# Allenxuxu/gev

Measured on AMD Instinct MI355X. Metric: GiB/s WS payload unmasked (device-resident) + frames/s, 64 KiB masked frames, higher is better.
Workload: dtype u8

## Files before the change

### gev_amd/csrc/gevws_kernels.hpp

```cpp
#pragma once

#include <hip/hip_runtime.h>

#include <cstdint>
#include <cstdio>
#include <cstring>

#include "gevws.h"

typedef uint32_t u32x4 __attribute__((ext_vector_type(4)));
typedef uint64_t u64x2 __attribute__((ext_vector_type(2)));

namespace {

constexpr int kWalkBlock = 256;
constexpr int kCountBlock = 64;
constexpr int kScanBlock = 1024;
constexpr int kUnmaskBlock = 256;
constexpr uint64_t kTile = GEVWS_TILE;
static_assert(kTile == kUnmaskBlock * 16, "one tile = one 16-byte chunk per lane");
constexpr int kBlkFields = 4;
constexpr int kDecFields = 5;
constexpr uint32_t kFusedScanMaxBlocks = 256;
constexpr size_t kWalkPartBytes = (size_t)kFusedScanMaxBlocks * kDecFields * 2 * sizeof(uint64_t);
// ... 269 lines not shown
constexpr uint32_t kSmallConns = 256;
constexpr uint64_t kSmallBytes = 64 * 1024;
constexpr uint32_t kOneLaunchConns = GEVWS_ONE_LAUNCH_MAX_CONNS;
constexpr uint64_t kOneLaunchBytes = GEVWS_ONE_LAUNCH_MAX_BYTES;
static_assert(kOneLaunchConns == 1024 && kOneLaunchBytes == 128 * 1024, "k_decode_small's wide shape");
__device__ __forceinline__ uint64_t gpu_ticks() { return __builtin_amdgcn_s_memrealtime(); }
__device__ __forceinline__ void signal_done(uint32_t* done, uint32_t seq, uint64_t* ticks = nullptr, uint64_t t0 = 0,
                                            int slot = 0) {
  if (!done) return;
  if (ticks && threadIdx.x == 0) {
    ticks[2 * slot] = t0;
    ticks[2 * slot + 1] = gpu_ticks();
  }
  __threadfence_system();
  __syncthreads();
  if (threadIdx.x == 0) __hip_atomic_store(done, seq, __ATOMIC_RELEASE, __HIP_MEMORY_SCOPE_SYSTEM);
}

constexpr uint64_t kSplitMinBytes = 16384;
constexpr uint32_t kSplitMaxLanes = 32;
constexpr uint64_t kSplitLanesPerCU = 512;

constexpr uint64_t kBigFrameBytes = 48 * 1024;
constexpr uint32_t kWideGridPerCU = 32;
constexpr uint64_t kWideGridTiles = 2ull << 20;
constexpr uint32_t kUnmaskRunCounters = 8;
constexpr uint64_t kUnmaskRun = 16;
constexpr uint64_t kUnmaskRunMinTiles = 64;

__device__ __forceinline__ uint32_t active_groups(uint64_t total, uint64_t nframes, uint32_t big_grid,
                                                  bool wide = false) {
  const uint32_t ncu = big_grid & 0xffffu, norm = big_grid >> 16;
  if (ncu == 0 || gridDim.x <= ncu || nframes == 0) return gridDim.x;
  if (total / nframes >= kBigFrameBytes) return ncu;
  return (norm == 0 || wide || gridDim.x <= norm) ? gridDim.x : norm;
}

template <bool NT>
__device__ __forceinline__ u32x4 ld16u_stream(const uint8_t* p) {
  if constexpr (NT) {
    return __builtin_nontemporal_load(reinterpret_cast<const u32x4*>(p));
  } else {
    return ld16u(p);
  }
}

__device__ __forceinline__ void st16_nt(uint8_t* p, u32x4 x) {
  __builtin_nontemporal_store(x, reinterpret_cast<u32x4*>(p));
}

constexpr int kWinTiles = 4;

__device__ __forceinline__ u32x4 rot_next_lane(u32x4 x) {
  return u32x4{(uint32_t)__builtin_amdgcn_update_dpp(0, (int)x[0], 0x134, 0xf, 0xf, false),
               (uint32_t)__builtin_amdgcn_update_dpp(0, (int)x[1], 0x134, 0xf, 0xf, false),
               (uint32_t)__builtin_amdgcn_update_dpp(0, (int)x[2], 0x134, 0xf, 0xf, false),
               (uint32_t)__builtin_amdgcn_update_dpp(0, (int)x[3], 0x134, 0xf, 0xf, false)};
}

__device__ __forceinline__ u32x4 funnel16(u32x4 a, u32x4 b, uint32_t m) {
  const uint32_t r = m & 3;
  u32x4 o;
  switch (m >> 2) {
    case 0:
      o = u32x4{__builtin_amdgcn_alignbyte(a[1], a[0], r), __builtin_amdgcn_alignbyte(a[2], a[1], r),
                __builtin_amdgcn_alignbyte(a[3], a[2], r), __builtin_amdgcn_alignbyte(b[0], a[3], r)};
      break;
    case 1:
      o = u32x4{__builtin_amdgcn_alignbyte(a[2], a[1], r), __builtin_amdgcn_alignbyte(a[3], a[2], r),
                __builtin_amdgcn_alignbyte(b[0], a[3], r), __builtin_amdgcn_alignbyte(b[1], b[0], r)};
      break;
    case 2:
      o = u32x4{__builtin_amdgcn_alignbyte(a[3], a[2], r), __builtin_amdgcn_alignbyte(b[0], a[3], r),
                __builtin_amdgcn_alignbyte(b[1], b[0], r), __builtin_amdgcn_alignbyte(b[2], b[1], r)};
      break;
    default:
      o = u32x4{__builtin_amdgcn_alignbyte(b[0], a[3], r), __builtin_amdgcn_alignbyte(b[1], b[0], r),
                __builtin_amdgcn_alignbyte(b[2], b[1], r), __builtin_amdgcn_alignbyte(b[3], b[2], r)};
      break;
  }
  return o;
}

}
```

### gev_amd/csrc/gevws_unmask.hip

```cpp
#include "gevws_internal.hpp"

namespace {

__device__ __forceinline__ uint64_t find_frame(const gevws_frame* __restrict__ frames,
                                               const uint32_t* __restrict__ tile_first, uint64_t t,
                                               uint64_t ntiles, uint64_t nframes, uint64_t p) {
  uint64_t lo = tile_first[t];
  uint64_t hi = (t + 1 < ntiles) ? (uint64_t)tile_first[t + 1] : nframes - 1;
  while (lo < hi) {
    const uint64_t mid = (lo + hi + 1) >> 1;
    if (frames[mid].payload_off <= p) lo = mid; else hi = mid - 1;
  }
  return lo;
}

__device__ __forceinline__ void unmask_chunk_lookup(const uint8_t* __restrict__ in,
                                                    const gevws_frame* __restrict__ frames,
                                                    const uint32_t* __restrict__ tile_first, uint64_t t,
                                                    uint64_t ntiles, uint64_t nframes, uint64_t p,
                                                    uint8_t* __restrict__ out) {
  const gevws_frame* fr = frames + find_frame(frames, tile_first, t, ntiles, nframes, p);
  const uint64_t rel = p - fr->payload_off;
  uint32_t k;
  memcpy(&k, fr->hdr.mask, 4);
// ... 155 lines not shown
    const uint64_t wbase = base;
    const uint64_t f_lo = tile_first[t];
    const uint64_t f_hi = wend_t < ntiles ? (uint64_t)tile_first[wend_t] : nframes - 1;
    const uint64_t F = f_hi - f_lo + 1;
    if (F <= (uint64_t)kWinFrames) {
      __syncthreads();
      for (uint64_t i = threadIdx.x; i < F; i += kUnmaskBlock) {
        const uint64_t* rec = reinterpret_cast<const uint64_t*>(frames + f_lo + i);
        const uint64_t w0 = rec[0];
        const uint64_t Ln = rec[1];
        const uint64_t po = rec[2];
        const uint64_t so = rec[3];
        s_start[i] = po > wbase ? (uint32_t)(po - wbase) : 0u;
        const uint64_t lend = po + Ln;
        s_lend[i] = lend <= wbase ? 0 : (lend - wbase > 0x7fffffffull ? 0x7fffffff : (int32_t)(lend - wbase));
        s_delta[i] = so - po;
        s_key[i] = ((w0 >> 24) & 0xff) ? (uint32_t)(w0 >> 32) : 0u;
      }
      __syncthreads();
      u32x4 v[WT];
      uint32_t key[WT];
      int32_t rem[WT];
#pragma unroll
      for (int u = 0; u < WT; ++u) {
        const uint32_t rel = (uint32_t)(u * kTile) + lane_off;
        const uint64_t p = wbase + rel;
        rem[u] = 0;
        key[u] = 0;
        v[u] = u32x4{0, 0, 0, 0};
        if ((uint64_t)u < wt && p < total) {
          uint32_t lo = 0, hi = (uint32_t)F - 1;
          while (lo < hi) {
            const uint32_t mid = (lo + hi + 1) >> 1;
            if (s_start[mid] <= rel) lo = mid; else hi = mid - 1;
          }
          rem[u] = s_lend[lo] - (int32_t)rel;
          key[u] = s_key[lo];
          v[u] = ld16u_stream<true>(in + (p + s_delta[lo]));
        }
      }
#pragma unroll
      for (int u = 0; u < WT; ++u) {
        if (rem[u] > 0) {
          u32x4 x = v[u] ^ key[u];
          if (rem[u] < 16) x = keep_bytes(x, rem[u]);
          st16_nt(out + wbase + (uint32_t)(u * kTile) + lane_off, x);
        }
      }
      t = wend_t;
      continue;
    }
    const uint64_t p = base + lane_off;
    if (p < total) unmask_chunk_lookup(in, frames, tile_first, t, ntiles, nframes, p, out);
    t += 1;
  }
  if (!dyn) break;
  }
}

constexpr int kWin5Frames = 1024;
constexpr uint32_t kWinChunks = 8 * (uint32_t)kTile / 16;
constexpr uint32_t kQuarter = kWinChunks / (kUnmaskBlock / 64);
constexpr uint32_t kTmapN = 512;

struct WinRec {
  u64x2 lo;
  u64x2 hi;
};

__device__ __forceinline__ WinRec load_rec(const gevws_frame* __restrict__ frames, uint64_t f) {
  const u64x2* r = reinterpret_cast<const u64x2*>(frames + f);
  return WinRec{r[0], r[1]};
}

struct WinLds5 {
  int32_t* lend;
  uint64_t* delta;
  uint32_t* key;
  uint16_t* own;
  uint32_t* wtot;
  uint32_t* tmap;
};

template <int U>
__device__ __forceinline__ void unmask_v5_body(const uint8_t* __restrict__ in, const gevws_frame* __restrict__ frames,
                                               const uint32_t* __restrict__ tile_first,
                                               const gevws_summary* __restrict__ sum, uint8_t* __restrict__ out,
                                               uint32_t big_grid, const WinLds5& L, bool wide = false,
                                               uint32_t* __restrict__ runs = nullptr) {
  constexpr int WT = 8;
  static_assert(WT * kTile / 16 == kWinChunks && kWinChunks == 8 * kUnmaskBlock, "8 chunks per thread");
  if (sum->status != GEVWS_OK) return;
  const uint64_t total = sum->payload_bytes;
  const uint64_t nframes = sum->frames;
  const uint64_t ntiles = (total + kTile - 1) / kTile;
  const uint32_t groups = active_groups(total, nframes, big_grid, wide);
  if (blockIdx.x >= groups) return;
  const uint64_t per = (ntiles + groups - 1) / groups;
  const bool dyn = runs != nullptr && groups >= kUnmaskRunCounters;
  uint64_t t = dyn ? 0 : (uint64_t)blockIdx.x * per;
  uint64_t tend = dyn ? 0 : (t + per < ntiles ? t + per : ntiles);
  const uint32_t xc = blockIdx.x % kUnmaskRunCounters;
  const uint64_t segn = ((ntiles + kUnmaskRunCounters - 1) / kUnmaskRunCounters + kUnmaskRun - 1) / kUnmaskRun * kUnmaskRun;
  const uint64_t seg0 = xc * segn < ntiles ? xc * segn : ntiles;
  const uint64_t seg1 = seg0 + segn < ntiles ? seg0 + segn : ntiles;
  {
    const uint32_t tid = fresh_tid();
    reinterpret_cast<u32x4*>(L.own)[tid] = u32x4{0, 0, 0, 0};
    reinterpret_cast<u32x4*>(L.own + kWinChunks)[tid] = u32x4{0, 0, 0, 0};
    if (tid < 2 * (kUnmaskBlock / 64)) L.wtot[tid] = 0;
  }
  __syncthreads();
  uint64_t f_po = 0, f_end = 0, f_src = 0;
  int64_t f_len = 0;
  uint32_t f_key = 0;
  uint64_t pf_t = ~0ull, pf_a = 0, pf_b = 0;
  bool pf_stream = false;
  WinRec r0 = {};
  uint32_t buf = 0;
  uint64_t tm0 = ~0ull;
  auto cache_frame = [&](uint64_t f) {
    const uint64_t* rec = reinterpret_cast<const uint64_t*>(frames + f);
    const uint64_t w0 = uniform64(rec[0]);
    f_len = (int64_t)uniform64(rec[1]);
    f_po = uniform64(rec[2]);
    f_src = uniform64(rec[3]);
    f_end = f_po + round16((uint64_t)f_len);
    f_key = ((w0 >> 24) & 0xff) ? (uint32_t)(w0 >> 32) : 0u;
  };
  auto tmap_at = [&](uint64_t x) -> uint64_t {
    if (tm0 == ~0ull || x < tm0 || x + 16 >= tm0 + kTmapN) {
      __syncthreads();
      tm0 = x;
      for (uint32_t i = fresh_tid(); i < kTmapN; i += kUnmaskBlock) {
        const uint64_t y = x + i;
        L.tmap[i] = y < ntiles ? tile_first[y] : 0u;
      }
      __syncthreads();
    }
    return uniform32(L.tmap[x - tm0]);
  };
  auto decide = [&](uint64_t x, uint64_t& a, uint64_t& b, bool& stream) {
    a = tmap_at(x);
    stream = false;
    if (x + U <= tend && tmap_at(x + U - 1) == a) {
      cache_frame(a);
      stream = x * kTile >= f_po && (x + U) * kTile <= f_end;
    }
    const uint64_t wt = (tend - x) < (uint64_t)WT ? (tend - x) : (uint64_t)WT;
    b = x + wt < ntiles ? tmap_at(x + wt) : nframes - 1;
  };
  for (;;) {
  if (dyn) {
    __syncthreads();
    if (threadIdx.x == 0) L.tmap[kTmapN] = atomicAdd(runs + xc * 16, 1u);
    __syncthreads();
    t = seg0 + (uint64_t)L.tmap[kTmapN] * kUnmaskRun;
    if (t >= seg1) break;
    tend = t + kUnmaskRun < seg1 ? t + kUnmaskRun : seg1;
    pf_t = ~0ull;
    r0 = WinRec{};
  }
  while (t < tend) {
    const uint64_t base = t * kTile;
    if (t + U <= tend && base >= f_po && base + U * kTile <= f_end) {
      stream_step<U>(in, out, base, f_po, f_src, f_len, f_key);
      t += U;
      pf_t = ~0ull;
      r0 = WinRec{};
      continue;
    }
    uint64_t a, b;
    bool stream, have = false;
    if (pf_t == t) {
      a = pf_a;
      b = pf_b;
      stream = pf_stream;
      have = !pf_stream;
    } else {
      decide(t, a, b, stream);
    }
    if (stream) {
      stream_step<U>(in, out, base, f_po, f_src, f_len, f_key);
      t += U;
      pf_t = ~0ull;
      r0 = WinRec{};
      continue;
    }
    const uint64_t wt = (tend - t) < (uint64_t)WT ? (tend - t) : (uint64_t)WT;
    const uint64_t wend_t = t + wt;
    const uint64_t wbase = base;
    const uint64_t F = b - a + 1;
    if (F > (uint64_t)kWin5Frames) {
      const uint64_t p = base + fresh_tid() * 16;
      if (p < total) unmask_chunk_lookup(in, frames, tile_first, t, ntiles, nframes, p, out);
      t += 1;
      pf_t = ~0ull;
      r0 = WinRec{};
      continue;
    }
    uint16_t* const own = L.own + buf * kWinChunks;
    uint32_t* const carry = L.wtot + buf * (kUnmaskBlock / 64);
    __syncthreads();
    auto fill = [&](uint64_t i, const WinRec& q) {
      const uint64_t Ln = q.lo[1], po = q.hi[0], so = q.hi[1];
      const uint64_t lend = po + Ln;
      L.lend[i] = lend <= wbase ? 0 : (lend - wbase > 0x7fffffffull ? 0x7fffffff : (int32_t)(lend - wbase));
      L.delta[i] = so - po;
      L.key[i] = ((q.lo[0] >> 24) & 0xff) ? (uint32_t)(q.lo[0] >> 32) : 0u;
      if (Ln) {
        const uint64_t sc = po > wbase ? (po - wbase) >> 4 : 0;
        if (sc < kWinChunks) own[sc] = (uint16_t)(i + 1);
        const uint64_t ec = (po + round16(Ln) - wbase) >> 4;
#pragma unroll
        for (uint32_t w = 1; w < kUnmaskBlock / 64; ++w)
          if (sc < w * kQuarter && w * kQuarter < ec) carry[w] = (uint32_t)(i + 1);
      }
    };
    const uint32_t tid = fresh_tid();
    if (tid < F) fill(tid, have ? r0 : load_rec(frames, a + tid));
    for (uint64_t i = tid + kUnmaskBlock; i < F; i += kUnmaskBlock) fill(i, load_rec(frames, a + i));
    __syncthreads();
    {
      const uint32_t j = fresh_tid(), lane = j & 63, w = j >> 6;
      u32x4 m = reinterpret_cast<const u32x4*>(own)[j];
      uint32_t run[8];
#pragma unroll
      for (int k = 0; k < 4; ++k) {
        run[2 * k] = m[k] & 0xffffu;
        run[2 * k + 1] = m[k] >> 16;
      }
#pragma unroll
      for (int k = 1; k < 8; ++k) run[k] = run[k] > run[k - 1] ? run[k] : run[k - 1];
      uint32_t inc = run[7];
#pragma unroll
      for (int d = 1; d < 64; d <<= 1) {
        const uint32_t y = (uint32_t)__shfl_up((int)inc, d, 64);
        if (lane >= (uint32_t)d) inc = inc > y ? inc : y;
      }
      uint32_t exc = (uint32_t)__shfl_up((int)inc, 1, 64);
      const uint32_t seed = w ? carry[w] : 0u;
      if (lane == 0) exc = 0;
      exc = exc > seed ? exc : seed;
#pragma unroll
      for (int k = 0; k < 4; ++k) {
        const uint32_t lo16 = run[2 * k] > exc ? run[2 * k] : exc;
        const uint32_t hi16 = run[2 * k + 1] > exc ? run[2 * k + 1] : exc;
        m[k] = lo16 | (hi16 << 16);
      }
      reinterpret_cast<u32x4*>(own)[j] = m;
      reinterpret_cast<u32x4*>(L.own + (buf ^ 1) * kWinChunks)[j] = u32x4{0, 0, 0, 0};
      if (lane == 0) L.wtot[(buf ^ 1) * (kUnmaskBlock / 64) + w] = 0;
    }
    u32x4 v[WT];
    uint32_t key[WT];
    int32_t rem[WT];
    uint32_t lov[WT];
#pragma unroll
    for (int u = 0; u < WT; ++u) {
      const uint32_t tq = fresh_tid();
      const uint32_t c = (tq >> 6) * kQuarter + (uint32_t)u * 64 + (tq & 63);
      const uint32_t o = own[c];
      lov[u] = o ? o - 1 : 0;
    }
    const uint32_t tl = fresh_tid();
    const uint32_t loff = (tl >> 6) * kQuarter * 16 + (tl & 63) * 16;
#pragma unroll
    for (int u = 0; u < WT; ++u) {
      const uint32_t rel = (uint32_t)u * 1024 + loff;
      const uint64_t p = wbase + rel;
      rem[u] = 0;
      key[u] = 0;
      v[u] = u32x4{0, 0, 0, 0};
      if ((uint64_t)rel < wt * kTile && p < total) {
        const uint32_t lo = lov[u];
        rem[u] = L.lend[lo] - (int32_t)rel;
        key[u] = L.key[lo];
        v[u] = ld16u_stream<true>(in + (p + L.delta[lo]));
      }
    }
    __asm__ volatile("" ::: "memory");
    pf_t = ~0ull;
    if (wend_t < tend) {
      decide(wend_t, pf_a, pf_b, pf_stream);
      pf_t = wend_t;
      if (!pf_stream) {
        const uint64_t nF = pf_b - pf_a + 1;
        const uint32_t tid2 = fresh_tid();
        if (tid2 < nF) r0 = load_rec(frames, pf_a + tid2);
      }
    }
    const uint32_t ts = fresh_tid();
    const uint32_t soff = (ts >> 6) * kQuarter * 16 + (ts & 63) * 16;
#pragma unroll
    for (int u = 0; u < WT; ++u) {
      if (rem[u] > 0) {
        u32x4 x = v[u] ^ key[u];
        if (rem[u] < 16) x = keep_bytes(x, rem[u]);
        st16_nt(out + wbase + (uint32_t)u * 1024 + soff, x);
      }
    }
    buf ^= 1;
    t = wend_t;
  }
  if (!dyn) break;
  }
}

__global__ __launch_bounds__(kUnmaskBlock) __attribute__((amdgpu_waves_per_eu(4))) void k_unmask_auto5(
    const uint8_t* __restrict__ in, const gevws_frame* __restrict__ frames, const uint32_t* __restrict__ tile_first,
    const gevws_summary* __restrict__ sum, uint8_t* __restrict__ out, uint32_t big_grid, uint32_t* __restrict__ runs) {
  static_assert(kWinFrames == kWin5Frames, "one frame table for both bodies");
  __shared__ uint32_t s_start[kWinFrames];
  __shared__ int32_t s_lend[kWinFrames];
  __shared__ uint64_t s_delta[kWinFrames];
  __shared__ uint32_t s_key[kWinFrames];
  __shared__ __attribute__((aligned(16))) uint16_t s_own[2 * kWinChunks];
  __shared__ uint32_t s_wtot[2 * (kUnmaskBlock / 64)];
  __shared__ uint32_t s_tmap[kTmapN + 1];
  if (2 * sum->run_frames >= sum->frames)
    unmask_v3_body<16>(in, frames, tile_first, sum, out, big_grid, WinLds{s_start, s_lend, s_delta, s_key}, runs,
                       s_tmap + kTmapN);
  else
    unmask_v5_body<16>(in, frames, tile_first, sum, out, big_grid,
                       WinLds5{s_lend, s_delta, s_key, s_own, s_wtot, s_tmap},
                       sum->payload_bytes / kTile < kWideGridTiles, runs);
}

__global__ __launch_bounds__(kUnmaskBlock) __attribute__((amdgpu_waves_per_eu(4))) void k_unmask_v5(
    const uint8_t* __restrict__ in, const gevws_frame* __restrict__ frames, const uint32_t* __restrict__ tile_first,
    const gevws_summary* __restrict__ sum, uint8_t* __restrict__ out, uint32_t big_grid, uint32_t* __restrict__ runs) {
  __shared__ int32_t s_lend[kWin5Frames];
  __shared__ uint64_t s_delta[kWin5Frames];
  __shared__ uint32_t s_key[kWin5Frames];
  __shared__ __attribute__((aligned(16))) uint16_t s_own[2 * kWinChunks];
  __shared__ uint32_t s_wtot[2 * (kUnmaskBlock / 64)];
  __shared__ uint32_t s_tmap[kTmapN + 1];
  unmask_v5_body<16>(in, frames, tile_first, sum, out, big_grid,
                     WinLds5{s_lend, s_delta, s_key, s_own, s_wtot, s_tmap},
                     sum->payload_bytes / kTile < kWideGridTiles, runs);
}

__global__ __launch_bounds__(256) void k_cipher(uint8_t* __restrict__ p, uint64_t n, uint32_t key,
                                                uint64_t offset, uint64_t nchunks) {
  const uint64_t a0 = reinterpret_cast<uint64_t>(p) & ~uint64_t(15);
  const uint64_t pe = reinterpret_cast<uint64_t>(p) + n;
  const uint32_t s = (uint32_t)((offset - reinterpret_cast<uint64_t>(p)) & 3);
  const uint32_t krot = s ? ((key >> (8 * s)) | (key << (32 - 8 * s))) : key;
  for (uint64_t k = (uint64_t)blockIdx.x * blockDim.x + threadIdx.x; k < nchunks;
       k += (uint64_t)gridDim.x * blockDim.x) {
    const uint64_t a = a0 + 16 * k;
    if (a >= reinterpret_cast<uint64_t>(p) && a + 16 <= pe) {
      u32x4* q = reinterpret_cast<u32x4*>(a);
      *q = *q ^ krot;
    } else {
      for (uint32_t b = 0; b < 16; ++b) {
        const uint64_t x = a + b;
        if (x >= reinterpret_cast<uint64_t>(p) && x < pe) {
          const uint32_t idx = (uint32_t)((offset + (x - reinterpret_cast<uint64_t>(p))) & 3);
          *reinterpret_cast<uint8_t*>(x) ^= (uint8_t)(key >> (8 * idx));
        }
      }
    }
  }
}

using UnmaskFn = void (*)(const uint8_t*, const gevws_frame*, const uint32_t*, const gevws_summary*, uint8_t*,
                         uint32_t, uint32_t*);
struct UnmaskVariant {
  UnmaskFn fn;
  int unroll;
  const char* name;
  bool wide = false;
  bool runs = true;
};
const UnmaskVariant kUnmaskVariants[] = {
    {k_unmask_auto5, 16,
     "auto: v3 4-tile windows for batches of equal-size frames, v5 (pipelined 8-tile windows with a chunk -> frame "
     "map and the tile map cached in LDS) otherwise; non-temporal streaming and window loads; a wide grid for a "
     "smaller batch of mixed sizes after one on this context", true},
    {k_unmask_v5, 16, "v5 for every batch (the default's mixed-batch path alone)", true},
    {k_unmask_auto5, 16, "the default with one contiguous run per workgroup on the v5 path (rounds 1-3; measurement)",
     true, false},
};
constexpr int kNumUnmaskVariants = sizeof(kUnmaskVariants) / sizeof(kUnmaskVariants[0]);

}

namespace gevws_impl {

int unmask_variant_count() { return kNumUnmaskVariants; }
const char* unmask_variant_name(int i) { return i >= 0 && i < kNumUnmaskVariants ? kUnmaskVariants[i].name : nullptr; }

int launch_unmask(gevws_ctx* ctx, hipStream_t st, uint64_t payload_cap, const uint8_t* d_in,
                  const gevws_frame* d_frames, const uint32_t* tile_first, const gevws_summary* d_summary,
                  uint8_t* d_payload) {
  const UnmaskVariant& v = kUnmaskVariants[ctx->unmask_variant];
  const uint64_t ntiles = (payload_cap + kTile - 1) / kTile;
  const uint32_t ucus = (uint32_t)ctx->num_cus;
  const uint64_t norm = 4 * (uint64_t)ucus;
  const bool wide = v.wide && !ctx->unmask_grid && ctx->stats_known && ctx->prev_mixed &&
                    ntiles < kWideGridTiles && norm <= 0xffffu;
  uint64_t grid = ctx->unmask_grid ? (uint64_t)ctx->unmask_grid : wide ? kWideGridPerCU * (uint64_t)ucus : norm;
  const uint64_t useful = (ntiles + v.unroll - 1) / v.unroll;
  if (grid > useful) grid = useful;
  if (grid < 1) grid = 1;
  ctx->last_unmask_grid = (uint32_t)grid;
  v.fn<<<(uint32_t)grid, kUnmaskBlock, 0, st>>>(d_in, d_frames, tile_first, d_summary, d_payload,
                                                ctx->unmask_grid ? 0u : ucus | (wide ? (uint32_t)norm << 16 : 0u),
                                                v.runs ? ctx->unmask_runs : nullptr);
  return GEVWS_OK;
}

}

using namespace gevws_impl;

extern "C" {

int gevws_copy_async(gevws_ctx* ctx, void* stream, uint8_t* d_dst, const uint8_t* d_src, uint64_t n,
                     uint32_t grid) {
  if (!ctx || (n && (!d_dst || !d_src))) return GEVWS_ERR_INVALID;
  if (grid & 0x80000000u) return GEVWS_ERR_INVALID;
  const bool plain = grid & 0x40000000u, wspan = grid & 0x20000000u, pstore = grid & 0x10000000u,
             anyal = pstore || (grid & 0x08000000u);
  if ((n & 15) || (!anyal && (reinterpret_cast<uint64_t>(d_dst) & 15))) return GEVWS_ERR_INVALID;
  if (n == 0) return GEVWS_OK;
  DeviceGuard g(ctx->device);
  hipStream_t st = pick_stream(ctx, stream);
  grid &= 0x07ffffffu;
  if (grid == 0) grid = (uint32_t)ctx->num_cus;
  auto k = pstore ? (plain ? k_copy_stream<16, false, false, true> : k_copy_stream<16, true, false, true>)
           : wspan ? (plain ? k_copy_stream<16, false, true> : k_copy_stream<16, true, true>)
                   : (plain ? k_copy_stream<16, false, false> : k_copy_stream<16, true, false>);
  k<<<grid, kUnmaskBlock, 0, st>>>(d_src, d_dst, n);
  GEVWS_HIP(hipGetLastError());
  return GEVWS_OK;
}

int gevws_cipher_async(gevws_ctx* ctx, void* stream, uint8_t* d_p, uint64_t n, const uint8_t mask[4],
                       uint64_t offset) {
  if (!ctx || !mask || (n && !d_p)) return GEVWS_ERR_INVALID;
  if (n == 0) return GEVWS_OK;
  DeviceGuard g(ctx->device);
  hipStream_t st = pick_stream(ctx, stream);
  uint32_t key;
  memcpy(&key, mask, 4);
  const uint64_t a0 = reinterpret_cast<uint64_t>(d_p) & ~uint64_t(15);
  const uint64_t nchunks = (reinterpret_cast<uint64_t>(d_p) + n - a0 + 15) / 16;
  uint64_t grid = (nchunks + 255) / 256;
  if (grid > 4096) grid = 4096;
  k_cipher<<<(uint32_t)grid, 256, 0, st>>>(d_p, n, key, offset, nchunks);
  GEVWS_HIP(hipGetLastError());
  return GEVWS_OK;
}

}
```

### gev_amd/csrc/gevws_walk.hip

```cpp
#include <chrono>

#include "gevws_internal.hpp"
#include "gevws_small.hpp"

namespace {

__device__ __forceinline__ void put_partial(uint64_t* part, uint32_t b, int k, uint64_t v, uint32_t tag) {
  uint64_t* p = part + 2 * ((uint64_t)b * kDecFields + k);
  put_granule(p, (uint32_t)v, tag);
  put_granule(p + 1, (uint32_t)(v >> 32), tag);
}

__device__ void scan_partials_wave(const uint64_t* __restrict__ part, uint32_t tag, uint64_t* __restrict__ blk,
                                   uint32_t nblk, uint64_t max_frames, uint64_t payload_cap,
                                   gevws_summary* __restrict__ sum) {
  constexpr int P = 4;
  const int lane = threadIdx.x & 63;
  uint64_t carry[kDecFields] = {0, 0, 0, 0, 0};
  uint32_t bad = 0;
  for (uint64_t base = 0; base < nblk; base += 64 * P) {
    const uint64_t i0 = base + (uint64_t)lane * P;
    uint64_t g[P][kDecFields][2];
#pragma unroll
    for (int r = 0; r < P; ++r)
// ... 194 lines not shown
      const uint64_t next = pos + fsz;
      load_window(s + (next <= len ? next : len), nlo, nhi);
      const uint64_t avail = len - pos;
      const bool have_hdr = avail >= 6 && avail >= hlen;
      const bool msb = e64 && (L64 >> 63);
      if (!have_hdr || msb || avail - hlen < L) {
        if (have_hdr && msb) { st = GEVWS_ERR_LEN_MSB; err += 1; }
        return false;
      }
      const uint32_t key = (e64 ? (uint32_t)(chi >> 16) : (e16 ? (uint32_t)(clo >> 32) : (uint32_t)(clo >> 16))) &
                           (0u - masked);
      const uint32_t meta = ((uint32_t)clo & 0xffu) | (masked << 8) | (hlen << 16);
      put_entry(key, L, meta);
      pos = next;
      if constexpr (D > 0) {
        run = fsz == prev_fsz ? run + 1 : 1;
        prev_fsz = fsz;
        if (run >= 3) {
          bool fail = false;
          for (;;) {
            uint64_t qlo[D], qhi[D];
            uint32_t qn = 1;
#pragma unroll
            for (int j = 1; j < D; ++j) {
              const uint64_t q = pos + (uint64_t)j * fsz;
              const bool in = q <= len;
              qn += in ? 1u : 0u;
              load_window(s + (in ? q : len), qlo[j], qhi[j]);
            }
            qlo[0] = nlo;
            qhi[0] = nhi;
            bool stop = false;
#pragma unroll
            for (int j = 0; j < D; ++j) {
              if (!stop && (uint32_t)j < qn) {
                uint32_t m2, h2, k2;
                uint64_t L2;
                const int r = walk_parse(qlo[j], qhi[j], len - pos, m2, h2, L2, k2);
                if (r != GEVWS_OK) {
                  if (r == GEVWS_ERR_LEN_MSB) { st = GEVWS_ERR_LEN_MSB; err += 1; }
                  fail = stop = true;
                } else {
                  put_entry(k2, L2, m2);
                  pos += h2 + L2;
                  if (h2 + L2 != fsz) {
                    stop = true;
                    run = 1;
                    prev_fsz = h2 + L2;
                  }
                }
              }
            }
            if (fail) break;
            load_window(s + pos, nlo, nhi);
            if (stop || qn < (uint32_t)D || pos + fsz > len) break;
          }
          if (fail) return false;
          if constexpr (ST == 0) *sink = WalkEntry{0, 0};
        }
      }
      return true;
    };
    uint64_t lo2 = 0, hi2 = 0;
    for (;;) {
      if (!step(lo, hi, lo2, hi2)) break;
      if (!step(lo2, hi2, lo, hi)) break;
    }
    R.pos = pos;
    R.nf = nf;
    R.pb = pb;
    R.pl = pl;
    R.same = same;
    R.lastf = lastf;
    R.firstf = firstf;
    R.err = err;
    R.st = st;
    R.rec = rec;
    if constexpr (ST == 2) {
      __asm__ volatile("" ::: "memory");
      lds_st(ring.head, (uint32_t)nf | kRingDone);
    }
}

template <uint32_t GROUP = kWriterGroup, uint32_t RING = kRing>
__device__ __forceinline__ void walk_ring_writer(WalkEntry* __restrict__ entries, WalkRing ring, uint64_t ebase,
                                                 uint64_t ecap) {
  static_assert(GROUP <= kSlotAlign && kSlotAlign % GROUP == 0 && RING % GROUP == 0 && GROUP % 4 == 0,
                "groups aligned by the slot runs, whole groups in the ring");
  uint32_t t = 0;
  bool fin = false;
  for (;;) {
    if (!fin) {
      const uint32_t hv = lds_ld(ring.head);
      __asm__ volatile("" ::: "memory");
      const uint32_t h = hv & ~kRingDone;
      while (h - t >= GROUP) {
        WalkEntry g[GROUP];
#pragma unroll
        for (uint32_t k = 0; k < GROUP; ++k) g[k] = ring.e[(t + k) & (RING - 1)];
        if (ebase != ~0ull && t + GROUP <= ecap) {
          u32x4* d = reinterpret_cast<u32x4*>(entries + ebase + t);
#pragma unroll
          for (uint32_t k = 0; k < GROUP / 2; ++k)
            d[k] = u32x4{g[2 * k].mask, g[2 * k].w, g[2 * k + 1].mask, g[2 * k + 1].w};
        }
        t += GROUP;
        __asm__ volatile("" ::: "memory");
        lds_st(ring.tail, t);
      }
      if (hv & kRingDone) {
        for (; t < h; ++t)
          if (ebase != ~0ull && t < ecap) entries[ebase + t] = ring.e[t & (RING - 1)];
        fin = true;
      }
    }
    if (__all(fin)) break;
    __builtin_amdgcn_s_sleep(2);
  }
}

template <int D, int ST>
__global__ __launch_bounds__(ST == 2 ? 2 * kCountBlock : kCountBlock) void k_walk_count(
    const uint8_t* __restrict__ in, const gevws_conn_in* __restrict__ conns, uint32_t n,
    gevws_conn_out* __restrict__ cout, uint64_t* __restrict__ blk, WalkEntry* __restrict__ entries, uint64_t n_entries,
    uint32_t gshift, uint32_t cpb, uint64_t in_bytes, uint32_t* __restrict__ done, uint64_t* __restrict__ part,
    uint32_t tag, uint64_t max_frames, uint64_t payload_cap, gevws_summary* __restrict__ sum) {
  __shared__ WalkEntry s_ring[ST == 2 ? kCountBlock * kRing : 1];
  __shared__ uint32_t s_head[ST == 2 ? kCountBlock : 1], s_tail[ST == 2 ? kCountBlock : 1];
  __shared__ uint64_t s_ebase[ST == 2 ? kCountBlock : 1], s_ecap[ST == 2 ? kCountBlock : 1];
  const uint32_t lane = threadIdx.x & 63;
  const bool walker = ST != 2 || threadIdx.x < 64;
  const uint32_t c = blockIdx.x * cpb + lane;
  const bool active = walker && lane < cpb && c < n;
  uint64_t nf = 0, pb = 0, pl = 0, err = 0, same = 0;
  gevws_conn_in ci = {0, 0};
  int32_t st = GEVWS_OK;
  uint64_t ebase = 0, ecap = 0;
  bool rec0 = false;
  if (active) {
    ci = conns[c];
    if (out_of_order(conns, c, ci)) err = 1ull << 32;
    if (ci.off > in_bytes || ci.len > in_bytes - ci.off) {
      ci.off = 0;
      ci.len = 0;
      st = GEVWS_ERR_INVALID;
      err += 1;
    }
    rec0 = entry_slots_of(ci, c, n_entries, gshift, ebase, ecap);
  }
  const WalkRing ring = {s_ring + lane * kRing, s_head + lane, s_tail + lane};
  if constexpr (ST == 2) {
    if (walker) {
      s_head[lane] = active ? 0u : kRingDone;
      s_tail[lane] = 0;
      s_ebase[lane] = rec0 ? ebase : ~0ull;
      s_ecap[lane] = ecap;
    }
    __syncthreads();
    if (!walker) walk_ring_writer(entries, ring, s_ebase[lane], s_ecap[lane]);
  }
  if (active) {
    WalkRes R = walk_res_fresh(err, st);
    walk_chain<D, ST>(in + ci.off, ci.len, rec0, ebase, ecap, entries, entries + n_entries + c, R, ring);
    nf = R.nf;
    pb = R.pb;
    pl = R.pl;
    err = R.err;
    same = R.same;
    gevws_conn_out o;
    o.first_frame = R.rec ? 1 : 0;
    o.consumed = R.pos;
    o.payload_base = pb;
    o.nframes = (uint32_t)nf;
    o.status = R.st;
    cout[c] = o;
  }
  const uint64_t vals[kDecFields] = {nf, pb, pl, err, same};
#pragma unroll
  for (int k = 0; k < kDecFields; ++k) {
    const uint64_t s = wave_sum(vals[k]);
    if (threadIdx.x == 0) {
      if (done) put_partial(part, blockIdx.x, k, s, tag);
      else blk[(uint64_t)blockIdx.x * kDecFields + k] = s;
    }
  }
  if (done) walk_block_done(done, gridDim.x, part, tag, blk, max_frames, payload_cap, sum, threadIdx.x == 0);
}

constexpr uint32_t kSyncWin = 256;
constexpr uint32_t kSyncRow = kSyncWin / 4 + 5;
constexpr int kSyncDepth = 5;
constexpr uint32_t kSplitAutoMaxLanes = 16;
constexpr uint64_t kSplitMinFramesPerConn = 256;
constexpr uint64_t kSplitMaxConnsPerCU = 64;
constexpr uint64_t kSplitMaxFrameBytes = 4096;

__device__ __forceinline__ bool sync_plausible1(uint32_t b0, uint32_t b1, uint32_t m0) {
  const uint32_t op = b0 & 0x0fu;
  const bool data = op <= 2, ctrl = op >= 8 && op <= 10;
  return (b0 & 0x70u) == 0 && (b1 >> 7) == m0 && (data || (ctrl && (b0 & 0x80u) && (b1 & 0x7fu) <= 125));
}

__device__ __forceinline__ uint64_t sync_frame(uint64_t lo, uint64_t hi, uint64_t rem, uint32_t m0) {
  const uint32_t b0 = (uint32_t)lo & 0xffu, b1 = (uint32_t)(lo >> 8) & 0xffu;
  if (!sync_plausible1(b0, b1, m0)) return 0;
  const uint32_t len7 = b1 & 0x7fu;
  const uint32_t hlen = 2 + (len7 == 127 ? 8u : (len7 == 126 ? 2u : 0u)) + 4 * (b1 >> 7);
  uint64_t L = len7;
  if (len7 == 126) {
    L = (((lo >> 16) & 0xff) << 8) | ((lo >> 24) & 0xff);
// ... 96 lines not shown
    }
    if (ok && lb < qmax) {
      b = lb;
      return true;
    }
  }
  return false;
}

constexpr uint32_t kSplitRing = 32;
constexpr uint32_t kSplitGroup = 16;
constexpr uint32_t kSplitLdsWords = (kCountBlock * kSyncRow > 2 * kCountBlock * kSplitRing)
                                        ? kCountBlock * kSyncRow
                                        : 2 * kCountBlock * kSplitRing;

template <int KS, int D, int ST>
__global__ __launch_bounds__(ST == 2 ? 2 * kCountBlock : kCountBlock) void k_walk_split(const uint8_t* __restrict__ in,
                                                            const gevws_conn_in* __restrict__ conns, uint32_t n,
                                                            gevws_conn_out* __restrict__ cout,
                                                            uint64_t* __restrict__ blk,
                                                            WalkEntry* __restrict__ entries, uint64_t n_entries,
                                                            uint32_t gshift, uint32_t cpb, uint64_t in_bytes,
                                                            uint32_t* __restrict__ done,
                                                            uint64_t* __restrict__ part, uint32_t tag,
                                                            uint64_t max_frames,
                                                            uint64_t payload_cap, gevws_summary* __restrict__ sum,
                                                            gevws_conn_in* __restrict__ segs,
                                                            gevws_conn_out* __restrict__ sout,
                                                            uint8_t* __restrict__ srec,
                                                            uint64_t min_seg = kSplitMinBytes,
                                                            uint32_t* __restrict__ fallbacks = nullptr) {
  static_assert(KS >= 2 && KS <= (int)kSplitMaxLanes && (KS & (KS - 1)) == 0, "KS: a power of two");
  static_assert(ST == 0 || ST == 2, "entries from the lanes or through the writer wave");
  __shared__ __attribute__((aligned(16))) uint32_t s_lds[ST == 2 ? kSplitLdsWords : kCountBlock * kSyncRow];
  __shared__ uint32_t s_head[ST == 2 ? kCountBlock : 1], s_tail[ST == 2 ? kCountBlock : 1];
  __shared__ uint64_t s_ebase[ST == 2 ? kCountBlock : 1], s_ecap[ST == 2 ? kCountBlock : 1];
  uint32_t* const s_row = s_lds;
  const bool walker = ST != 2 || threadIdx.x < 64;
  const uint32_t lane = threadIdx.x & 63, i = lane % KS;
  const uint32_t c = blockIdx.x * cpb + lane / KS;
  const bool active = walker && lane / KS < cpb && c < n;
  const uint64_t v = (uint64_t)c * KS + i;
  gevws_conn_in ci = {0, 0};
  bool oob = false;
  if (active) {
    ci = conns[c];
    oob = ci.off > in_bytes || ci.len > in_bytes - ci.off;
    if (oob) ci = gevws_conn_in{0, 0};
  }
  const uint8_t* s = in + ci.off;
  bool found = active && i == 0;
  uint64_t b = 0;
  if (active && i > 0) {
    const uint64_t kc = ci.len / min_seg < KS ? ci.len / min_seg : KS;
    if (i < kc) {
      const uint64_t seg = ci.len / kc, t = ci.len * i / kc;
      const uint64_t step = seg / (2 * kSyncWindows) > kSyncWin ? seg / (2 * kSyncWindows) : kSyncWin;
      const uint32_t m0 = (uint32_t)s[1] >> 7;
      found = sync_search(s, ci.len, t, step, t + seg * 3 / 4, m0, s_row + lane * kSyncRow, b);
    }
  }
  const uint64_t mine = found ? b : ~0ull;
  uint64_t end = ci.len;
#pragma unroll
  for (int j = KS - 1; j >= 1; --j) {
    const uint64_t y = __shfl(mine, (int)((lane + j) & 63), 64);
    if ((int)i + j < KS && y != ~0ull) end = y;
  }
  const uint64_t sb = found ? b : end;
  const uint64_t slen = found ? end - b : 0;
  gevws_conn_in sg = {ci.off + sb, slen};
  uint64_t ebase = 0, ecap = 0;
  const bool rec0 = active && entry_slots_of(sg, (uint32_t)v, n_entries, gshift, ebase, ecap);
  WalkRes R = walk_res_fresh();
  if constexpr (ST == 2) {
    const WalkRing ring = {reinterpret_cast<WalkEntry*>(s_lds) + lane * kSplitRing, s_head + lane, s_tail + lane};
    if (walker) {
      s_head[lane] = active ? 0u : kRingDone;
      s_tail[lane] = 0;
      s_ebase[lane] = rec0 ? ebase : ~0ull;
      s_ecap[lane] = ecap;
    }
    __syncthreads();
    if (!walker) walk_ring_writer<kSplitGroup, kSplitRing>(entries, ring, s_ebase[lane], s_ecap[lane]);
    else if (active)
      walk_chain<D, 2, kSplitRing>(in + sg.off, sg.len, rec0, ebase, ecap, entries, entries + n_entries + v, R, ring);
  } else if (active) {
    walk_chain<D>(in + sg.off, sg.len, rec0, ebase, ecap, entries, entries + n_entries + v, R);
  }
  const bool last = found && end == ci.len;
  const bool ok = !found || last || (R.st == GEVWS_OK && R.pos == slen);
  uint64_t prevlast = ~0ull;
  bool got = false;
#pragma unroll
  for (int d = 1; d < KS; ++d) {
    const uint64_t ynf = __shfl_up(R.nf, d, 64), ylast = __shfl_up(R.lastf, d, 64);
    if (!got && (int)i >= d && ynf > 0) {
      prevlast = ylast;
      got = true;
    }
  }
  const uint64_t same = R.same + ((R.nf > 0 && got && R.firstf == prevlast) ? 1 : 0);
  uint64_t inf = R.nf, ipb = R.pb;
#pragma unroll
  for (int d = 1; d < KS; d <<= 1) {
    const uint64_t a = __shfl_up(inf, d, 64), q = __shfl_up(ipb, d, 64);
    if ((int)i >= d) {
      inf += a;
      ipb += q;
    }
  }
  uint64_t t_nf = R.nf, t_pb = R.pb, t_pl = R.pl, t_same = same;
  uint64_t t_cons = last ? sb + R.pos : 0;
  int32_t t_st = last ? R.st : 0;
  int t_ok = ok ? 1 : 0;
#pragma unroll
  for (int d = KS / 2; d >= 1; d >>= 1) {
    t_nf += __shfl_xor(t_nf, d, 64);
    t_pb += __shfl_xor(t_pb, d, 64);
    t_pl += __shfl_xor(t_pl, d, 64);
    t_same += __shfl_xor(t_same, d, 64);
    t_cons += __shfl_xor(t_cons, d, 64);
    t_st += __shfl_xor(t_st, d, 64);
    t_ok &= __shfl_xor(t_ok, d, 64);
  }
  const bool valid = t_ok != 0 && !oob;
  uint64_t nf = 0, pb = 0, pl = 0, err = 0, rs = 0;
  if (active) {
    if (valid) {
      segs[v] = sg;
      gevws_conn_out so;
      so.first_frame = inf - R.nf;
      so.consumed = R.pos;
      so.payload_base = ipb - R.pb;
      so.nframes = (uint32_t)R.nf;
      so.status = R.st;
      sout[v] = so;
      srec[v] = R.rec ? 1 : 0;
    }
    if (i == 0) {
      gevws_conn_out o;
      o.first_frame = 0;
      if (oob) {
        o.consumed = 0;
        o.payload_base = 0;
        o.nframes = 0;
        o.status = GEVWS_ERR_INVALID;
      } else if (valid) {
        nf = t_nf;
        pb = t_pb;
        pl = t_pl;
        rs = t_same;
        o.consumed = t_cons;
        o.payload_base = pb;
        o.nframes = (uint32_t)nf;
        o.status = t_st;
      } else {
        if (fallbacks) atomicAdd(fallbacks, 1u);
        WalkRes S = walk_res_fresh();
        walk_chain<0>(s, ci.len, false, 0, 0, entries, entries + n_entries + v, S);
        nf = S.nf;
        pb = S.pb;
        pl = S.pl;
        rs = S.same;
        o.consumed = S.pos;
        o.payload_base = pb;
        o.nframes = (uint32_t)nf;
// ... 704 lines not shown
```

Measured before the change: 2947.

## Align v5 window loads and realign in registers; cooperative line writes in walk writer

The v5 unmask path now rounds each chunk's unaligned source address down to a 16-byte boundary when the frame's bytes allow it. It recovers the payload by funnel-shifting across neighbouring lanes' registers, which avoids split unaligned global loads. The walk ring writer gains a mode where lanes of a wave cooperate to copy whole entry groups as 16-byte stores, replacing the per-lane scalar group copies. Both add cross-lane shuffles and selection logic that cost extra ALU work and complexity, and the old unaligned path is kept as a measurement variant.

After: 2491. 0.845x the previous value.

```diff
diff --git a/gev_amd/csrc/gevws_kernels.hpp b/gev_amd/csrc/gevws_kernels.hpp
--- a/gev_amd/csrc/gevws_kernels.hpp
+++ b/gev_amd/csrc/gevws_kernels.hpp
@@ -375,4 +375,14 @@
   return o;
 }
 
-}
+__device__ __forceinline__ u32x4 funnel16_lane(u32x4 a, u32x4 b, uint32_t m) {
+  const uint32_t r = m & 3;
+  const bool q1 = m & 4, q2 = m & 8;
+  const uint32_t t0 = q1 ? a[1] : a[0], t1 = q1 ? a[2] : a[1], t2 = q1 ? a[3] : a[2], t3 = q1 ? b[0] : a[3],
+                 t4 = q1 ? b[1] : b[0], t5 = q1 ? b[2] : b[1], t6 = q1 ? b[3] : b[2];
+  const uint32_t s0 = q2 ? t2 : t0, s1 = q2 ? t3 : t1, s2 = q2 ? t4 : t2, s3 = q2 ? t5 : t3, s4 = q2 ? t6 : t4;
+  return u32x4{__builtin_amdgcn_alignbyte(s1, s0, r), __builtin_amdgcn_alignbyte(s2, s1, r),
+               __builtin_amdgcn_alignbyte(s3, s2, r), __builtin_amdgcn_alignbyte(s4, s3, r)};
+}
+
+}
diff --git a/gev_amd/csrc/gevws_unmask.hip b/gev_amd/csrc/gevws_unmask.hip
--- a/gev_amd/csrc/gevws_unmask.hip
+++ b/gev_amd/csrc/gevws_unmask.hip
@@ -261,7 +261,7 @@
   uint32_t* tmap;
 };
 
-template <int U>
+template <int U, bool AL>
 __device__ __forceinline__ void unmask_v5_body(const uint8_t* __restrict__ in, const gevws_frame* __restrict__ frames,
                                                const uint32_t* __restrict__ tile_first,
                                                const gevws_summary* __restrict__ sum, uint8_t* __restrict__ out,
@@ -428,7 +428,9 @@
         m[k] = lo16 | (hi16 << 16);
       }
       reinterpret_cast<u32x4*>(own)[j] = m;
-      reinterpret_cast<u32x4*>(L.own + (buf ^ 1) * kWinChunks)[j] = u32x4{0, 0, 0, 0};
+      uint32_t z = 0;
+      __asm__ volatile("" : "+v"(z));
+      reinterpret_cast<u32x4*>(L.own + (buf ^ 1) * kWinChunks)[j] = u32x4{z, z, z, z};
       if (lane == 0) L.wtot[(buf ^ 1) * (kUnmaskBlock / 64) + w] = 0;
     }
     u32x4 v[WT];
@@ -444,6 +446,10 @@
     }
     const uint32_t tl = fresh_tid();
     const uint32_t loff = (tl >> 6) * kQuarter * 16 + (tl & 63) * 16;
+    const uint32_t qend = ((tl >> 6) + 1) * kQuarter * 16;
+    const bool whole = (uint64_t)qend <= wt * kTile;
+    const uint32_t send = whole ? qend : (uint32_t)(wt * kTile);
+    u32x4 e = u32x4{0, 0, 0, 0};
 #pragma unroll
     for (int u = 0; u < WT; ++u) {
       const uint32_t rel = (uint32_t)u * 1024 + loff;
@@ -453,9 +459,21 @@
       v[u] = u32x4{0, 0, 0, 0};
       if ((uint64_t)rel < wt * kTile && p < total) {
         const uint32_t lo = lov[u];
-        rem[u] = L.lend[lo] - (int32_t)rel;
+        const int32_t rb = L.lend[lo] - (int32_t)rel;
+        rem[u] = rb < 0 ? 0 : (rb > 16 ? 16 : rb);
         key[u] = L.key[lo];
-        v[u] = ld16u_stream<true>(in + (p + L.delta[lo]));
+        const uint8_t* a = in + (p + L.delta[lo]);
+        if constexpr (AL) {
+          const uint32_t mis = (uint32_t)(reinterpret_cast<uint64_t>(a) & 15);
+          const bool ends = rel + (uint32_t)rb <= send;
+          const bool ok = ends ? mis + (((uint32_t)rb - 1) & 15) < 16 : whole;
+          if (rb > 0 && mis != 0 && ok && a - mis >= in) {
+            rem[u] |= (int32_t)(mis << 8);
+            a -= mis;
+            if (u == WT - 1 && !ends && (tl & 63) == 63) e = ld16u_stream<true>(a + 16);
+          }
+        }
+        v[u] = ld16u_stream<true>(a);
       }
     }
     __asm__ volatile("" ::: "memory");
@@ -471,11 +489,20 @@
     }
     const uint32_t ts = fresh_tid();
     const uint32_t soff = (ts >> 6) * kQuarter * 16 + (ts & 63) * 16;
+    u32x4 rn = u32x4{0, 0, 0, 0};
+    if constexpr (AL) rn = rot_next_lane(v[0]);
 #pragma unroll
     for (int u = 0; u < WT; ++u) {
-      if (rem[u] > 0) {
-        u32x4 x = v[u] ^ key[u];
-        if (rem[u] < 16) x = keep_bytes(x, rem[u]);
+      u32x4 x = v[u];
+      if constexpr (AL) {
+        const u32x4 r = rn;
+        rn = u + 1 < WT ? rot_next_lane(v[u + 1 < WT ? u + 1 : u]) : e;
+        x = funnel16_lane(x, (ts & 63) == 63 ? rn : r, (uint32_t)rem[u] >> 8);
+      }
+      const int32_t rb = rem[u] & 0xff;
+      if (rb > 0) {
+        x = x ^ key[u];
+        if (rb < 16) x = keep_bytes(x, rb);
         st16_nt(out + wbase + (uint32_t)u * 1024 + soff, x);
       }
     }
@@ -486,6 +513,7 @@
   }
 }
 
+template <bool AL>
 __global__ __launch_bounds__(kUnmaskBlock) __attribute__((amdgpu_waves_per_eu(4))) void k_unmask_auto5(
     const uint8_t* __restrict__ in, const gevws_frame* __restrict__ frames, const uint32_t* __restrict__ tile_first,
     const gevws_summary* __restrict__ sum, uint8_t* __restrict__ out, uint32_t big_grid, uint32_t* __restrict__ runs) {
@@ -501,9 +529,9 @@
     unmask_v3_body<16>(in, frames, tile_first, sum, out, big_grid, WinLds{s_start, s_lend, s_delta, s_key}, runs,
                        s_tmap + kTmapN);
   else
-    unmask_v5_body<16>(in, frames, tile_first, sum, out, big_grid,
-                       WinLds5{s_lend, s_delta, s_key, s_own, s_wtot, s_tmap},
-                       sum->payload_bytes / kTile < kWideGridTiles, runs);
+    unmask_v5_body<16, AL>(in, frames, tile_first, sum, out, big_grid,
+                           WinLds5{s_lend, s_delta, s_key, s_own, s_wtot, s_tmap},
+                           sum->payload_bytes / kTile < kWideGridTiles, runs);
 }
 
 __global__ __launch_bounds__(kUnmaskBlock) __attribute__((amdgpu_waves_per_eu(4))) void k_unmask_v5(
@@ -515,9 +543,9 @@
   __shared__ __attribute__((aligned(16))) uint16_t s_own[2 * kWinChunks];
   __shared__ uint32_t s_wtot[2 * (kUnmaskBlock / 64)];
   __shared__ uint32_t s_tmap[kTmapN + 1];
-  unmask_v5_body<16>(in, frames, tile_first, sum, out, big_grid,
-                     WinLds5{s_lend, s_delta, s_key, s_own, s_wtot, s_tmap},
-                     sum->payload_bytes / kTile < kWideGridTiles, runs);
+  unmask_v5_body<16, true>(in, frames, tile_first, sum, out, big_grid,
+                           WinLds5{s_lend, s_delta, s_key, s_own, s_wtot, s_tmap},
+                           sum->payload_bytes / kTile < kWideGridTiles, runs);
 }
 
 __global__ __launch_bounds__(256) void k_cipher(uint8_t* __restrict__ p, uint64_t n, uint32_t key,
@@ -554,13 +582,17 @@
   bool runs = true;
 };
 const UnmaskVariant kUnmaskVariants[] = {
-    {k_unmask_auto5, 16,
+    {k_unmask_auto5<true>, 16,
      "auto: v3 4-tile windows for batches of equal-size frames, v5 (pipelined 8-tile windows with a chunk -> frame "
-     "map and the tile map cached in LDS) otherwise; non-temporal streaming and window loads; a wide grid for a "
+     "map and the tile map cached in LDS, its window loads aligned and realigned in registers where a frame's chunks "
+     "allow) otherwise; non-temporal streaming and window loads; a wide grid for a "
      "smaller batch of mixed sizes after one on this context", true},
     {k_unmask_v5, 16, "v5 for every batch (the default's mixed-batch path alone)", true},
-    {k_unmask_auto5, 16, "the default with one contiguous run per workgroup on the v5 path (rounds 1-3; measurement)",
+    {k_unmask_auto5<true>, 16, "the default with one contiguous run per workgroup on the v5 path (rounds 1-3; measurement)",
      true, false},
+    {k_unmask_auto5<false>, 16,
+     "the default with every v5 window load an unaligned 16-byte load at the chunk's own address (rounds 1-6; "
+     "measurement)", true},
 };
 constexpr int kNumUnmaskVariants = sizeof(kUnmaskVariants) / sizeof(kUnmaskVariants[0]);
 
diff --git a/gev_amd/csrc/gevws_walk.hip b/gev_amd/csrc/gevws_walk.hip
--- a/gev_amd/csrc/gevws_walk.hip
+++ b/gev_amd/csrc/gevws_walk.hip
@@ -300,18 +300,50 @@
     }
 }
 
-template <uint32_t GROUP = kWriterGroup, uint32_t RING = kRing>
+template <uint32_t GROUP = kWriterGroup, uint32_t RING = kRing, bool LINES = true>
 __device__ __forceinline__ void walk_ring_writer(WalkEntry* __restrict__ entries, WalkRing ring, uint64_t ebase,
                                                  uint64_t ecap) {
   static_assert(GROUP <= kSlotAlign && kSlotAlign % GROUP == 0 && RING % GROUP == 0 && GROUP % 4 == 0,
                 "groups aligned by the slot runs, whole groups in the ring");
+  constexpr uint32_t LPG = GROUP / 2;
+  constexpr uint32_t GPI = 64 / LPG;
+  static_assert(LPG * GPI == 64, "a group's lanes divide the wave");
+  const uint32_t lane = threadIdx.x & 63, sub = lane / LPG, piece = lane % LPG;
   uint32_t t = 0;
   bool fin = false;
   for (;;) {
+    uint32_t hv = 0, h = 0;
     if (!fin) {
-      const uint32_t hv = lds_ld(ring.head);
+      hv = lds_ld(ring.head);
       __asm__ volatile("" ::: "memory");
-      const uint32_t h = hv & ~kRingDone;
+      h = hv & ~kRingDone;
+    }
+    if constexpr (LINES) {
+      bool ready = !fin && h - t >= GROUP;
+      for (uint64_t m = __ballot(ready); m; m = __ballot(ready)) {
+        uint64_t s = m, rest = m;
+        __asm__ volatile("" ::: "memory");
+#pragma unroll
+        for (uint32_t k = 1; k < GPI; ++k) s = sub >= k ? s & (s - 1) : s;
+#pragma unroll
+        for (uint32_t k = 0; k < GPI; ++k) rest &= rest - 1;
+        const bool on = s != 0;
+        const uint32_t src = on ? (uint32_t)__builtin_ctzll(s) : lane;
+        const uint32_t ts = (uint32_t)__shfl((int)t, (int)src, 64);
+        const uint64_t eb = __shfl(ebase, (int)src, 64), ec = __shfl(ecap, (int)src, 64);
+        if (on && eb != ~0ull && ts + GROUP <= ec) {
+          const WalkEntry* r = ring.e + ((int32_t)src - (int32_t)lane) * (int32_t)RING;
+          const u32x4 x = *reinterpret_cast<const u32x4*>(r + ((ts + 2 * piece) & (RING - 1)));
+          *reinterpret_cast<u32x4*>(entries + eb + ts + 2 * piece) = x;
+        }
+        if (ready && !((rest >> lane) & 1)) {
+          t += GROUP;
+          __asm__ volatile("" ::: "memory");
+          lds_st(ring.tail, t);
+          ready = h - t >= GROUP;
+        }
+      }
+    } else if (!fin) {
       while (h - t >= GROUP) {
         WalkEntry g[GROUP];
 #pragma unroll
@@ -326,11 +358,11 @@
         __asm__ volatile("" ::: "memory");
         lds_st(ring.tail, t);
       }
-      if (hv & kRingDone) {
-        for (; t < h; ++t)
-          if (ebase != ~0ull && t < ecap) entries[ebase + t] = ring.e[t & (RING - 1)];
-        fin = true;
-      }
+    }
+    if (!fin && (hv & kRingDone)) {
+      for (; t < h; ++t)
+        if (ebase != ~0ull && t < ecap) entries[ebase + t] = ring.e[t & (RING - 1)];
+      fin = true;
     }
     if (__all(fin)) break;
     __builtin_amdgcn_s_sleep(2);
@@ -343,7 +375,7 @@
     gevws_conn_out* __restrict__ cout, uint64_t* __restrict__ blk, WalkEntry* __restrict__ entries, uint64_t n_entries,
     uint32_t gshift, uint32_t cpb, uint64_t in_bytes, uint32_t* __restrict__ done, uint64_t* __restrict__ part,
     uint32_t tag, uint64_t max_frames, uint64_t payload_cap, gevws_summary* __restrict__ sum) {
-  __shared__ WalkEntry s_ring[ST == 2 ? kCountBlock * kRing : 1];
+  __shared__ __attribute__((aligned(16))) WalkEntry s_ring[ST == 2 ? kCountBlock * kRing : 1];
   __shared__ uint32_t s_head[ST == 2 ? kCountBlock : 1], s_tail[ST == 2 ? kCountBlock : 1];
   __shared__ uint64_t s_ebase[ST == 2 ? kCountBlock : 1], s_ecap[ST == 2 ? kCountBlock : 1];
   const uint32_t lane = threadIdx.x & 63;
@@ -606,7 +638,7 @@
       s_ecap[lane] = ecap;
     }
     __syncthreads();
-    if (!walker) walk_ring_writer<kSplitGroup, kSplitRing>(entries, ring, s_ebase[lane], s_ecap[lane]);
+    if (!walker) walk_ring_writer<kSplitGroup, kSplitRing, false>(entries, ring, s_ebase[lane], s_ecap[lane]);
     else if (active)
       walk_chain<D, 2, kSplitRing>(in + sg.off, sg.len, rec0, ebase, ecap, entries, entries + n_entries + v, R, ring);
   } else if (active) {
```
